# kaiidams/voice100

Hardware: AMD Instinct MI355X
Metric: audio frames/sec (fwd+bwd) asr_en_base, B=32x1024-frame mel (higher is better)
Workload: dtype bf16

## Files before the change

include/voice100_hip.h:

```cpp
#ifndef VOICE100_HIP_H
#define VOICE100_HIP_H

#ifdef __cplusplus
extern "C" {
#endif


int v100_dw_num_groups(int B, int C);
int v100_dwconv(const float* x, const float* x2, const float* w, const float* in_a, const float* in_b,
                const float* in_c, int in_mode, float* y, const float* aux, const float* out_a,
                const float* out_b, int out_mode, float* stats, int G, int B, int C, int Tin, int Tout,
                int K, int stride, int pad, int flip, int upsample, int force_generic, void* stream);

int v100_dwconv_wgrad(const float* g, const float* g2, const float* ga, const float* gb, const float* gc,
                      int g_mode, const float* x, const float* xa, const float* xb, int x_mode,
                      float* partial, float* dw, int G, int B, int C, int Tin, int Tout, int K, int stride,
                      int pad, int force_generic, void* stream);

int v100_dwconv_bwd(const float* g, const float* g2, const float* w, const float* ga, const float* gb,
                    const float* gc, const float* xpre, const float* xa, const float* xb, float* dxin,
                    float* stats, float* wpartial, float* dw, int G, int B, int C, int Tin, int Tout, int K,
                    int stride, int pad, int force_split, void* stream);

int v100_pw_num_parts(int B, int T);
// ... 104 lines not shown
long long v100_launch_count(void);
int v100_copy_probe(const void* src, void* dst, long long nbytes, void* stream);
int v100_timing_enable(int tag_mask);
int v100_timing_read(int tag, double* ms, long long* count, double* bytes);
int v100_rows_copy_probe(const void* src, void* dst, int B, int C, int row_bytes, void* stream);

int v100_pw_gemm_io(const void* A_bf16, const void* X, const void* X2, const float* xa, const float* xb, const float* xc,
                    int x_mode, void* Y, const float* ea, const float* eb, const void* R, int epi_mode, float* stats,
                    int B, int M, int K, int T, int io16, void* stream);
int v100_pw_wgrad_io(const void* G, const void* G2, const float* ga, const float* gb, const float* gc, int g_mode,
                     const void* X, const float* xa, const float* xb, int x_mode, float* partial, float* dW, int S, int B,
                     int M, int K, int T, int io16, void* stream);
int v100_pw_wgrad_group_supported(int B, int M, int K, int T, int S, int g_mode, int x_mode, int io16);
int v100_pw_wgrad_group_tiles(int M, int K, int x_mode);
int v100_pw_wgrad_group(int n, const void* const* ptrs, const int* dims, void* stream);
int v100_dw_mfma_supported(int K, int stride);
int v100_row_pitch16(int T, int B);
int v100_dwconv_fwd_train_io(const void* a1, const float* w, const float* in_a, const float* in_b, void* a2, float* stats,
                             int G, int B, int C, int T, int K, int io16, void* stream);
int v100_dwconv_bwd_io(const void* g, const void* g2, const float* w, const float* ga, const float* gb, const float* gc,
                       const void* xpre, const float* xa, const float* xb, void* dxin, float* stats, float* wpartial,
                       float* dw, int G, int B, int C, int T, int K, int io16, void* stream);
int v100_dwconv_bwd_da1_io(const void* g, const void* g2, const float* w, const float* ga, const float* gb, const float* gc,
                           const void* xpre, const float* xa, const float* xb, void* da1_out, float* stats, float* dw,
                           const float* bn1_gamma, const float* bn1_mean, const float* bn1_rstd, float* pqr, float* dgamma,
                           float* dbeta, int B, int C, int T, int K, void* stream);
int v100_dwconv_fwd_eval_io(const void* h1, const float* w, const float* out_a, const float* out_b, void* h2, int B, int C, int T,
                            int K, int flags, void* stream);
int v100_chan_reduce2_io(const void* u, const void* v, float* partial, int G, int B, int C, int T, int io16, void* stream);
int v100_chan_affine2_shadow(const void* u, const float* v, const float* A, const float* Cc, float* out, void* shadow,
// ... 32 lines not shown
long long v100_ir_eval_cache_bytes(const int* shape);
int v100_ir_eval_prep(const int* shape, const void* const* ptrs, void* stream);
int v100_ir_fwd_eval(const int* shape, const void* const* ptrs, void* stream);
int v100_ir_stack_fwd_eval(int n, const int* shapes, const void* const* ptrs, void* stream);
int v100_ir_prep_batched(const int* shapes, const void* const* w1s, const void* const* w3s, void* const* preps, int n, void* stream);
int v100_ir_fwd_train(const int* shape, const void* const* ptrs, void* stream);
long long v100_ir_bwd_workspace_bytes(const int* shape);
int v100_ir_bwd(const int* shape, const void* const* ptrs, void* stream);

long long v100_ir_stack_plan(const int* desc, long long* plan);
int v100_ir_stack_fwd_train(const int* desc, const void* const* params, const void* x, const void* x16, void* blob, void* stream);
int v100_ir_stack_bwd(const int* desc, const void* const* params, const void* x, const void* x16, const void* blob, const void* dy,
                      void* dx, void* grads, void* ws, void* stream);
int v100_ir_stack_wgrad_plan(const int* desc, int have_x16, int min_problem_tiles, int min_flush_tiles, long long* out);
int v100_ir_stack_wgrad_group_thresholds(int min_problem_tiles, int min_flush_tiles);

int v100_ctc_greedy_decode(const float* logits, const int* lens, long long* out, int* out_len, int B, int T, int V, int blank, void* stream);
int v100_ctc_best_path(const float* logp, const long long* labels, const int* in_len, const int* lab_len, void* back_ws, int* path,
                       float* score, int B, int T, int V, int Lmax, int max_move, void* stream);
long long v100_ctc_align_workspace_bytes(int B, int T, int Lmax);
int v100_ctc_align_block(void);
int v100_ctc_align(const float* logp, const long long* labels, const int* in_len, const int* lab_len, void* moves_ws, int* path,
                   long long* best_labels, int* align, float* score, int B, int T, int V, int Lmax, int max_move, void* stream);
long long v100_edit_distance_workspace_bytes(int B, int Th, int Tr);
int v100_edit_distance(const long long* hyp, const int* hyp_len, const long long* ref, const int* ref_len, void* ws, int* dist,
                       int* hyp_n, int* ref_n, long long* totals, int B, int Th, int Tr, int levels, long long sep, void* stream);
long long v100_ctc_beam_workspace_bytes(int B, int T, int V, int W);
int v100_ctc_beam_search(const float* logits, const int* lens, void* ws, long long* ids, int* ids_len, float* scores, int B, int T, int V,
                         int W, int nbest, int blank, void* stream);
int v100_ctc_beam_search_lm(const float* logits, const int* lens, void* ws, long long* ids, int* ids_len, float* scores,
// ... 86 lines not shown
```

voice100_amd/csrc/block.hip:

```cpp
#include "common.h"
#include "../../include/voice100_hip.h"
#include "depthwise_common.h"
#include "block_shape.h"
#include <algorithm>

static inline size_t al256(size_t v) { return (v + 255) & ~size_t(255); }
static const float kMom = 0.1f, kEps = 1e-5f;
#define CK(call) do { rc = (call); if (rc) return rc; } while (0)

static inline int pitch16(int T, int B) { return v100_pitch16(T, B); }
extern "C" int v100_row_pitch16(int T, int B) { return v100_pitch16(T, B); }
enum { PW_IO_X = 1, PW_IO_X2 = 2, PW_IO_Y = 4, PW_IO_R = 8, PW_IO_F16 = 16, WG_IO_G = 1, WG_IO_G2 = 2, WG_IO_X = 4 };

struct IrBn { const float *gamma, *beta; float *rm, *rv; long long* nbt; };
struct IrBnCoef { float *s, *t, *m, *r; };
struct IrCoef { IrBnCoef bn1, bn2, bn3; };
static IrCoef ir_coef(const float* coef, int mc) {
    float* c = const_cast<float*>(coef);
    return {{c, c + mc, c + 2 * mc, c + 3 * mc}, {c + 4 * mc, c + 5 * mc, c + 6 * mc, c + 7 * mc}, {c + 8 * mc, c + 9 * mc, c + 10 * mc, c + 11 * mc}};
}
struct IrParams { const float* w1; IrBn bn1; const float* wd; IrBn bn2; const float* w3; IrBn bn3; };
static IrParams ir_params(const void* const* t) {
    auto bn = [&](int j) { return IrBn{(const float*)t[j], (const float*)t[j + 1], (float*)t[j + 2], (float*)t[j + 3], (long long*)t[j + 4]}; };
    return {(const float*)t[0], bn(1), (const float*)t[6], bn(7), (const float*)t[12], bn(13)};
// ... 114 lines not shown
    } else {
        w.dz2 = c.take<float>((size_t)B * hid * T2);
        w.dz1 = c.take<float>((size_t)B * hid * T);
    }
    w.slab = c.take<float>(std::max({(size_t)v100_pw_wgrad_splits(B, cout, hid) * cout * hid, (size_t)v100_pw_wgrad_splits(B, hid, cin) * hid * cin,
                                     (size_t)v100_dw_num_groups(B, hid) * hid * K}));
    w.pqr = c.take<float>((size_t)6 * s.mc);
    return c.used + 256;
}

static size_t ir_defer_da3_bytes(const IrShape& s) { return al256((size_t)s.B * s.cout * pitch16(s.T2, s.B) * 2); }
static size_t ir_defer_bytes(const IrShape& s) { return ir_defer_da3_bytes(s) + al256((size_t)s.B * s.hid * pitch16(s.T, s.B) * 2); }
static int ir_wgrad_defer_tiles(const IrShape& s) {
    return v100_pw_wgrad_group_tiles(s.cout, s.hid, 1) + v100_pw_wgrad_group_tiles(s.hid, s.cin, 0);
}
static bool ir_wgrad_defer_ok(const IrShape& s, bool have_x16, int min_tiles) {
    const int B = s.B, cin = s.cin, hid = s.hid, cout = s.cout, T = s.T, K = s.K;
    if (s.act16 < 4 || !s.shadows || s.frozen || !have_x16 || s.S != 1) return false;
    if (!ir_act16_supported(s) || v100_dw_num_groups(B, hid) != 1 || !dw_bwd_da1_supported(B, hid, T, K, 1)) return false;
    const int io = WG_IO_G | WG_IO_X;
    return v100_pw_wgrad_group_supported(B, cout, hid, T, v100_pw_wgrad_splits(B, cout, hid), 0, 1, io) &&
           v100_pw_wgrad_group_supported(B, hid, cin, T, v100_pw_wgrad_splits(B, hid, cin), 0, 0, io) &&
           v100_pw_wgrad_group_tiles(cout, hid, 1) >= min_tiles && v100_pw_wgrad_group_tiles(hid, cin, 0) >= min_tiles;
}

extern "C" long long v100_ir_bwd_workspace_bytes(const int* shape) {
    IrBwdWs w;
    IrShape s = ir_shape(shape, false);
    s.act16 = shape[IR_ACT16];
    return (long long)ir_bwd_carve(s, nullptr, w);
}

static int ir_bwd(const IrShape& s, const IrBwdArgs& a, hipStream_t stream) {
    const int B = s.B, cin = s.cin, hid = s.hid, cout = s.cout, T = s.T, K = s.K, S = s.S, res = s.res, bf = s.bf, pad = s.pad, T2 = s.T2, mc = s.mc;
    const float *x = a.x, *a1 = a.a1, *a2 = a.a2, *a3 = a.a3, *wd = a.wd, *g1 = a.g1, *g2 = a.g2, *g3 = a.g3, *dy = a.dy;
    const IrCoef c = ir_coef(a.coef, mc);
    const float *s1 = c.bn1.s, *t1 = c.bn1.t, *s2 = c.bn2.s, *t2 = c.bn2.t;
    float* dx = a.dx;
// ... 170 lines not shown
}
extern "C" int v100_ir_stack_fwd_eval(int n, const int* shapes, const void* const* ptrs, void* stream) {
    if (!shapes || !ptrs) return V100_ERR_NULL;
    if (n < 0) return V100_ERR_SHAPE;
    int rc;
    for (int i = 0; i < n; ++i, shapes += IR_NSHAPE, ptrs += 8)
        CK(ir_fwd_eval(ir_shape(shapes, false), ir_eval_layout(shapes), ir_eval_args(ptrs), (hipStream_t)stream));
    return V100_OK;
}

enum { ST_N, ST_B, ST_T, ST_BF16, ST_LEVEL, ST_SHADOW, ST_HDR };
namespace {
struct StackBlock { IrShape s; long long a1, a2, a3, y, y16, coef, prep; int Tout; size_t grad_floats; long long defer_off; };
struct StackTotals { size_t blob_bytes, bwd_ws, grad_floats, fwd_ws_off, wsmax, dxmax; };
int wg_min_problem_tiles = 32, wg_min_flush_tiles = 192;
int stack_layout(const int* desc, StackBlock* blk, StackTotals& t, int min_tiles = wg_min_problem_tiles) {
    t = StackTotals{};
    const int n = desc[ST_N], B = desc[ST_B], bf = desc[ST_BF16], level = desc[ST_LEVEL];
    if (n <= 0 || n > 32 || B <= 0 || desc[ST_T] <= 0 || (bf != 0 && bf != 1)) return 0;
    int T = desc[ST_T];
    size_t off = 0, fwd_ws = 0;
    const bool shadows = bf == 1 && level >= 4;
    for (int i = 0; i < n; ++i) {
        const int* d = desc + ST_HDR + 6 * i;
        StackBlock& b = blk[i];
        const int cin = d[0], hid = d[1], cout = d[2], k = d[3], st = d[4], res = d[5];
        if (cin <= 0 || hid <= 0 || cout <= 0 || k <= 0 || st <= 0) return 0;
        const int dims[9] = {B, cin, hid, cout, T, k, st, res, bf};
        IrShape& s = b.s = ir_shape(dims, false);
        s.prepped = true; s.shadows = shadows;
// ... 33 lines not shown
void stack_flush_plan(const StackBlock* blk, int n, bool have_x16, int min_flush, bool* defer, int* flush) {
    int tiles = 0, count = 0;
    for (int i = n - 1; i >= 0; --i) {
        defer[i] = blk[i].defer_off >= 0 && (i > 0 || have_x16);
        flush[i] = 0;
        if (defer[i]) { tiles += ir_wgrad_defer_tiles(blk[i].s); count += 2; }
        if (!count) continue;
        const bool next = i > 0 && blk[i - 1].defer_off >= 0 && (i > 1 || have_x16);
        const bool fits = next && count + 2 <= 16 && tiles + ir_wgrad_defer_tiles(blk[i - 1].s) <= 256;
        if (i == 0 || count + 2 > 16 || (tiles >= min_flush && !fits)) {
            flush[i] = tiles >= min_flush ? tiles : -tiles;
            tiles = count = 0;
        }
    }
}
}

extern "C" int v100_ir_stack_wgrad_group_thresholds(int min_problem_tiles, int min_flush_tiles) {
    if (min_problem_tiles < 1 || min_flush_tiles < 1) return V100_ERR_SHAPE;
    wg_min_problem_tiles = min_problem_tiles;
    wg_min_flush_tiles = min_flush_tiles;
    return V100_OK;
}

extern "C" int v100_ir_stack_wgrad_plan(const int* desc, int have_x16, int min_problem_tiles, int min_flush_tiles, long long* out) {
    if (!desc || !out) return V100_ERR_NULL;
    if (min_problem_tiles < 1 || min_flush_tiles < 1) return V100_ERR_SHAPE;
    StackBlock blk[32];
    StackTotals t;
    if (!stack_layout(desc, blk, t, min_problem_tiles)) return V100_ERR_SHAPE;
    const int n = desc[ST_N];
    bool defer[32]; int flush[32];
    stack_flush_plan(blk, n, have_x16 != 0, min_flush_tiles, defer, flush);
    size_t shared = t.bwd_ws;
    for (int i = 0; i < n; ++i) {
        out[3 * i] = defer[i]; out[3 * i + 1] = blk[i].defer_off; out[3 * i + 2] = flush[i];
        if (blk[i].defer_off >= 0 && (size_t)blk[i].defer_off < shared) shared = (size_t)blk[i].defer_off;
    }
    out[3 * n] = (long long)t.bwd_ws; out[3 * n + 1] = (long long)shared;
    return V100_OK;
}

extern "C" long long v100_ir_stack_plan(const int* desc, long long* plan) {
    if (!desc || !plan) return -1;
    StackBlock blk[32];
    StackTotals t;
    if (!stack_layout(desc, blk, t)) return -1;
    const int n = desc[ST_N];
    for (int i = 0; i < n; ++i) {
        long long* o = plan + 8 * i;
        o[0] = blk[i].a1; o[1] = blk[i].a2; o[2] = blk[i].a3; o[3] = blk[i].y; o[4] = blk[i].y16; o[5] = blk[i].coef; o[6] = blk[i].prep;
        o[7] = blk[i].Tout;
    }
    const long long tot[6] = {(long long)t.blob_bytes, (long long)t.bwd_ws, (long long)t.grad_floats, (long long)t.fwd_ws_off, 0, 0};
// ... 44 lines not shown
    const char* base = (const char*)blob;
    auto at = [&](long long off) { return (const float*)(base + off); };
    char* w0 = (char*)ws;
    char* pp[2] = {w0 + al256(t.wsmax), w0 + al256(t.wsmax) + al256(t.dxmax)};
    size_t goff = t.grad_floats;
    const void* dyi = dy;
    int rc;
    static const bool grad16_on = [] { const char* e = getenv("V100_IR_GRAD16"); return !(e && e[0] == '0'); }();
    auto grad16_ok = [&](int i) {
        const IrShape& s = blk[i].s;
        return grad16_on && desc[ST_LEVEL] >= 5 && s.act16 >= 3 && s.S == 1 && s.T >= 8 && chan_bn3_bwd_fits(s.B, s.T) && ir_act16_supported(s) &&
               dw_bwd_da1_supported(s.B, s.hid, s.T, s.K, v100_dw_num_groups(s.B, s.hid));
    };
    bool defer[32]; int flush[32];
    stack_flush_plan(blk, n, x16 != nullptr, wg_min_flush_tiles, defer, flush);
    const void* gp[5 * 16]; int gd[8 * 16]; int gblk[16]; int ng = 0;
    auto flush_pending = [&](bool grouped) -> int {
        int rc = V100_OK;
        if (grouped) rc = v100_pw_wgrad_group(ng, gp, gd, stream);
        else
            for (int j = 0; j < ng && rc == V100_OK; ++j) {
                IrBwdWs w;
                ir_bwd_carve(blk[gblk[j]].s, w0, w);
                const int* d = gd + 8 * j;
                rc = v100_pw_wgrad_io(gp[5 * j], nullptr, nullptr, nullptr, nullptr, d[5], gp[5 * j + 1], (const float*)gp[5 * j + 2],
                                      (const float*)gp[5 * j + 3], d[6], w.slab, (float*)const_cast<void*>(gp[5 * j + 4]), d[4], d[0], d[1], d[2], d[3],
                                      d[7], stream);
            }
        ng = 0;
        return rc;
    };
    bool dy_is16 = false;
    for (int i = n - 1; i >= 0; --i) {
        const StackBlock& b = blk[i];
        IrShape s = b.s;
        s.defer = defer[i];
        const bool dx_is16 = i > 0 && grad16_ok(i) && grad16_ok(i - 1);
        if (dy_is16 && !grad16_ok(i)) return V100_ERR_SHAPE;
        s.dy16 = dy_is16; s.dx16 = dx_is16;
        goff -= b.grad_floats;
        void* dxi = i > 0 ? (void*)pp[i & 1] : dx;
        const IrParams p = ir_params(params + 18 * i);
        const void* x16i = i > 0 ? (blk[i - 1].y16 >= 0 ? (const void*)(base + blk[i - 1].y16) : nullptr) : x16;
        IrBwdArgs a{i > 0 ? at(blk[i - 1].y) : (const float*)x, at(b.a1), at(b.a2), at(b.a3), p.w1, p.wd, p.w3, p.bn1.gamma, p.bn2.gamma, p.bn3.gamma,
                    at(b.coef), (const float*)dyi, (float*)dxi, {}, w0, (void*)(base + b.prep), x16i, defer[i] ? w0 + b.defer_off : nullptr};
        ir_grads_carve(s, (float*)grads + goff, a.g);
        CK(ir_bwd(s, a, (hipStream_t)stream));
        if (defer[i]) {
            const IrBnCoef bn2 = ir_coef(a.coef, s.mc).bn2;
            char* own = w0 + b.defer_off;
            const void* pr[2][5] = {{own, a.a2, bn2.s, bn2.t, a.g.dW3}, {own + ir_defer_da3_bytes(s), a.x16, nullptr, nullptr, a.g.dW1}};
            const int dm[2][8] = {{s.B, s.cout, s.hid, s.T, v100_pw_wgrad_splits(s.B, s.cout, s.hid), 0, 1, WG_IO_G | WG_IO_X},
                                  {s.B, s.hid, s.cin, s.T, v100_pw_wgrad_splits(s.B, s.hid, s.cin), 0, 0, WG_IO_G | WG_IO_X}};
            for (int j = 0; j < 2; ++j, ++ng) {
                for (int e = 0; e < 5; ++e) gp[5 * ng + e] = pr[j][e];
                for (int e = 0; e < 8; ++e) gd[8 * ng + e] = dm[j][e];
                gblk[ng] = i;
            }
        }
        if (flush[i]) CK(flush_pending(flush[i] > 0));
        dyi = dxi;
        dy_is16 = dx_is16;
    }
    return V100_OK;
}
```

voice100_amd/csrc/pointwise_bf16_group.hip:

```cpp
#include "pointwise_bf16_wgrad_group.h"
#include "timing.h"

extern "C" int v100_pw_wgrad_group_supported(int B, int M, int K, int T, int S, int g_mode, int x_mode, int io16) {
    if (B <= 0 || M <= 0 || K <= 0 || T <= 0 || S <= 0 || (S > B && (S % B != 0 || S / B > 64))) return 0;
    if (g_mode != PW_X_NONE || (x_mode != PW_X_NONE && x_mode != PW_X_AFFINE_RELU6) || io16 != (WG_IO_G | WG_IO_X)) return 0;
    const int GR = x_mode ? 256 : 128, XR = x_mode ? 128 : 256;
    if (M % GR || K % XR) return 0;
    const int P = pw_pitch16(T, B);
    return ((long)(M + 256) * P * 4 < 0x7fffffffL && (long)(K + 256) * P * 4 < 0x7fffffffL) ? 1 : 0;
}

extern "C" int v100_pw_wgrad_group_tiles(int M, int K, int x_mode) {
    const int GR = x_mode ? 256 : 128, XR = x_mode ? 128 : 256;
    return (M > 0 && K > 0 && M % GR == 0 && K % XR == 0) ? (M / GR) * (K / XR) : 0;
}

extern "C" int v100_pw_wgrad_group(int n, const void* const* ptrs, const int* dims, void* stream) {
    if (!ptrs || !dims) return V100_ERR_NULL;
    if (n <= 0 || n > WG_GROUP_MAX) return V100_ERR_SHAPE;
    WgGroupParams g;
    g.n = n;
    int fill[8] = {0, 0, 0, 0, 0, 0, 0, 0};
    bool tail = false;
    for (int i = 0; i < n; ++i) {
        const void* const* P = ptrs + 5 * i;
        const int* d = dims + 8 * i;
        if (!P[0] || !P[1] || !P[4] || (d[6] != PW_X_NONE && (!P[2] || !P[3]))) return V100_ERR_NULL;
        if (!v100_pw_wgrad_group_supported(d[0], d[1], d[2], d[3], d[4], d[5], d[6], d[7])) return V100_ERR_SHAPE;
        WgGroupProblem& q = g.pr[i];
        q.G = P[0]; q.X = P[1]; q.xa = (const float*)P[2]; q.xb = (const float*)P[3]; q.dW = (float*)P[4];
        q.B = d[0]; q.M = d[1]; q.K = d[2]; q.T = d[3]; q.S = d[4]; q.x_mode = d[6];
        q.ntiles = v100_pw_wgrad_group_tiles(q.M, q.K, q.x_mode);
        int x = 0;
        for (int c = 1; c < 8; ++c) if (fill[c] < fill[x]) x = c;
        q.xcd = x; q.slot0 = fill[x];
        fill[x] += q.ntiles;
        tail = tail || q.T % BF_BK != 0;
    }
    int slots = 0;
    for (int c = 0; c < 8; ++c) if (fill[c] > slots) slots = fill[c];
    hipStream_t st = (hipStream_t)stream;
    V100TimedRegion timed(V100_T_PW_WGRAD, st);
    if (tail) V100_GGL((pw_wgrad_group_kernel<true, WG_GROUP_RL>), dim3((unsigned)(8 * slots)), dim3(768), 0, st, g);
    else V100_GGL((pw_wgrad_group_kernel<false, WG_GROUP_RL>), dim3((unsigned)(8 * slots)), dim3(768), 0, st, g);
    return v100_launch_status();
}
```

voice100_amd/csrc/pointwise_bf16_wgrad_group.h:

```cpp
#pragma once
#include "pointwise_bf16_wgrad_ws.h"

struct WgGroupProblem {
    const void* G; const void* X; const float* xa; const float* xb; float* dW;
    int B, M, K, T, S, x_mode;
    int xcd, slot0, ntiles;
};
#define WG_GROUP_MAX 16
#define WG_GROUP_RL 2
struct WgGroupParams { WgGroupProblem pr[WG_GROUP_MAX]; int n; };

template <bool TAIL, int RL>
__global__ __launch_bounds__(768) void pw_wgrad_group_kernel(WgGroupParams g) {
    __shared__ __attribute__((aligned(16))) unsigned char smem[98304 + RL * 32768];
    const int x = blockIdx.x & 7, j = blockIdx.x >> 3;
    int pi = -1;
    for (int i = 0; i < g.n; ++i)
        if (g.pr[i].xcd == x && j >= g.pr[i].slot0 && j < g.pr[i].slot0 + g.pr[i].ntiles) pi = i;
    if (pi < 0) return;
    const WgGroupProblem& q = g.pr[pi];
    const int t = j - q.slot0;
    WgParams p{(const float*)q.G, nullptr, nullptr, nullptr, nullptr, (const float*)q.X, q.xa, q.xb, q.dW, q.B, q.M, q.K, q.T, q.S, 0, q.x_mode,
               0, 0, 0, 0, 0, 0, 0, 0u, WG_IO_G | WG_IO_X};
    f32x4* const runs = reinterpret_cast<f32x4*>(smem + 98304);
    if (q.x_mode == PW_X_AFFINE_RELU6) {
        const int nkt = q.K / 128;
        pw_wgrad_bf16_ws_body<0, 1, TAIL, WG_IO_G | WG_IO_X, 256, 128, 4, true, RL>(p, 0, t / nkt, t % nkt, smem, smem + 65536, runs);
    } else {
        const int nkt = q.K / 256;
        pw_wgrad_bf16_ws_body<0, 0, TAIL, WG_IO_G | WG_IO_X, 128, 256, 4, true, RL>(p, 0, t / nkt, t % nkt, smem, smem + 32768, runs);
    }
}
```

voice100_amd/csrc/pointwise_bf16_wgrad_ws.h:

```cpp
#pragma once
#include "pointwise_bf16_common.h"

template <int GM, int XM, bool TAIL, int IO, int GR, int XR, int NSW, bool GRP = false, int RL = 0>
__device__ __forceinline__ void pw_wgrad_bf16_ws_body(const WgParams& p, const int s, const int mt, const int ktile, unsigned char* const As0,
                                                      unsigned char* const Bs0, f32x4* const runs) {
    static_assert(!(GM != PW_X_NONE && XM != PW_X_NONE), "at most one transformed operand (128 rows); the other one plain (256 rows)");
    static_assert((IO & WG_IO_G) && (IO & WG_IO_X) && (GM != PW_X_AFFINE2 || (IO & WG_IO_G2)), "bf16-stored operands only");
    constexpr bool PG = GM == PW_X_NONE && XM != PW_X_NONE;
    static_assert((PG ? GR : XR) == 256 && (PG ? XR : GR) == 128, "tile shape");
    constexpr int QM = PG ? XM : GM;
    constexpr int NX = XR / 64;
    static_assert(NSW == 4 || NSW == 8, "staging waves: one or two per SIMD");
    constexpr int NSQ = (QM == PW_X_AFFINE2 && NSW == 4) ? 3 : 4;
    constexpr int NQP = 16 / NSW;
    constexpr int QRS = 8 * NSW;
    unsigned char (*As)[GR * 128] = reinterpret_cast<unsigned char (*)[GR * 128]>(As0);
    unsigned char (*Bs)[XR * 128] = reinterpret_cast<unsigned char (*)[XR * 128]>(Bs0);
    const int tid = threadIdx.x, lane = tid & 63;
    const int wave = __builtin_amdgcn_readfirstlane(tid >> 6);
    const int m0 = mt * GR, n0 = ktile * XR;
    const int M = p.M, K = p.K, T = p.T;
    const int P16 = pw_pitch16(T, p.B);
    const int nt = (T + BF_BK - 1) / BF_BK;
    const WgSpan sp = GRP ? WgSpan{0, p.B, 0, nt} : wg_span(p, s, nt);
    const int nsteps = sp.nb * sp.ntl, b_lo = sp.b_lo;
    auto step_bt = [&](int step, int& b, int& t0) {
// ... 1 lines not shown
        (void)q;
        const int bi = q / sp.ntl;
        b = b_lo + bi;
        t0 = (sp.t_first + q - bi * sp.ntl) * BF_BK;
    };
    auto tail_mask = [&](u32x4 v, int tb) {
        const int nv = T - tb;
#pragma unroll
        for (int j = 0; j < 4; ++j) v[j] &= nv > 2 * j + 1 ? 0xffffffffu : (nv > 2 * j ? 0xffffu : 0u);
        return v;
    };
    if (!GRP && nsteps == 0) {
        if (wave < 8) {
            const int wm = wave / NX, wn = wave % NX, col = lane & 31, half = lane >> 5;
#pragma unroll
            for (int i = 0; i < 2; ++i)
#pragma unroll
                for (int j = 0; j < 2; ++j)
#pragma unroll
                    for (int r = 0; r < 16; ++r) {
                        const int m = m0 + wm * 64 + i * 32 + (r & 3) + 8 * (r >> 2) + 4 * half, k = n0 + wn * 64 + j * 32 + col;
                        p.partial[((size_t)s * M + m) * K + k] = 0.f;
                    }
        }
        return;
    }

    if (wave >= 8) {
        const int pt = tid - 512;
        const int qrow = pt >> 3, ch = pt & 7;
        const int row0 = PG ? n0 : m0, rows = PG ? K : M;
        const float* q1 = PG ? p.X : p.G;
        const float* q2 = PG ? p.X : p.G2;
        const float* pa = PG ? p.xa : p.ga;
        const float* pb = PG ? p.xb : p.gb;
        unsigned char (*Qs)[128 * 128] = PG ? reinterpret_cast<unsigned char (*)[128 * 128]>(Bs) : reinterpret_cast<unsigned char (*)[128 * 128]>(As);
// ... 98 lines not shown
                    if (st + 2 < nsteps) {
                        stage(st + 3, S3{});
                        __syncthreads();
                    }
                }
            }
        }
#undef WS_SB
        return;
    }

    const int wm = wave / NX, wn = wave % NX;
    const int prow = tid >> 3, pch = tid & 7;
    const int prow0 = PG ? m0 : n0, prows = PG ? M : K;
    const float* pp = PG ? p.G : p.X;
    unsigned char (*Ps)[256 * 128] = PG ? reinterpret_cast<unsigned char (*)[256 * 128]>(As) : reinterpret_cast<unsigned char (*)[256 * 128]>(Bs);
    const int voP = ((prow0 + prow) * P16 + pch * 8) * 2;
    const int stepP = 64 * P16 * 2;
    const int ldsP = bf_off(prow, pch);
    u32x4 rp[2][4];
    auto load_p = [&](int step, auto stg, int i) {
        constexpr int SG = decltype(stg)::value;
        int b, t0;
        step_bt(step, b, t0);
        const __amdgpu_buffer_rsrc_t r = make_rsrc(reinterpret_cast<const u16*>(pp) + (size_t)b * prows * P16, (unsigned)prows * P16 * 2u);
        rp[SG][i] = __builtin_amdgcn_raw_buffer_load_b128(r, voP, t0 * 2 + i * stepP, 0);
    };
    auto piece_out = [&](int step, u32x4 v) {
        if constexpr (TAIL) {
            int b, t0;
            step_bt(step, b, t0);
            if (t0 + BF_BK > T) v = tail_mask(v, t0 + pch * 8);
        }
        return v;
    };
    f32x16 acc[2][2];
#pragma unroll
    for (int i = 0; i < 2; ++i)
#pragma unroll
        for (int j = 0; j < 2; ++j)
#pragma unroll
            for (int r = 0; r < 16; ++r) acc[i][j][r] = 0.f;
    const int lr = lane & 31, lh = lane >> 5;
    const int sw = (lr >> 1) & 7;
    const int rdA0 = (wm * 64 + lr) * 128, rdB0 = (wn * 64 + lr) * 128;
    auto block = [&](int st, auto stg) {
        constexpr int SG = decltype(stg)::value;
        const unsigned char* Ab = As[st & 1];
        const unsigned char* Bb = Bs[st & 1];
        unsigned char* Pd = Ps[(st + 1) & 1] + ldsP;
#pragma unroll
        for (int ks = 0; ks < BF_BK / 16; ++ks) {
            const int co = ((ks * 2 + lh) ^ sw) << 4;
            const bf16x8 a0 = *reinterpret_cast<const bf16x8*>(Ab + rdA0 + co);
            const bf16x8 a1 = *reinterpret_cast<const bf16x8*>(Ab + rdA0 + 32 * 128 + co);
            const bf16x8 b0 = *reinterpret_cast<const bf16x8*>(Bb + rdB0 + co);
            const bf16x8 b1 = *reinterpret_cast<const bf16x8*>(Bb + rdB0 + 32 * 128 + co);
            acc[0][0] = __builtin_amdgcn_mfma_f32_32x32x16_bf16(a0, b0, acc[0][0], 0, 0, 0);
            acc[0][1] = __builtin_amdgcn_mfma_f32_32x32x16_bf16(a0, b1, acc[0][1], 0, 0, 0);
            acc[1][0] = __builtin_amdgcn_mfma_f32_32x32x16_bf16(a1, b0, acc[1][0], 0, 0, 0);
            acc[1][1] = __builtin_amdgcn_mfma_f32_32x32x16_bf16(a1, b1, acc[1][1], 0, 0, 0);
            __builtin_amdgcn_sched_barrier(0);
            *reinterpret_cast<u32x4*>(Pd + ks * 8192) = piece_out(st + 1, rp[SG][ks]);
            load_p(st + 3, stg, ks);
            __builtin_amdgcn_sched_barrier(0);
        }
    };
    using S0 = std::integral_constant<int, 0>; using S1 = std::integral_constant<int, 1>;
#pragma unroll
    for (int i = 0; i < 4; ++i) load_p(0, S0{}, i);
    __builtin_amdgcn_sched_barrier(0);
#pragma unroll
    for (int i = 0; i < 4; ++i) load_p(1, S1{}, i);
    __builtin_amdgcn_sched_barrier(0);
#pragma unroll
    for (int i = 0; i < 4; ++i) { *reinterpret_cast<u32x4*>(Ps[0] + ldsP + i * 8192) = piece_out(0, rp[0][i]); load_p(2, S0{}, i); }
    __builtin_amdgcn_sched_barrier(0);
    __syncthreads();
    constexpr int NRR = GRP ? 4 - RL : 1;
    f32x16 run[NRR];
    const int per = ((p.B + p.S - 1) / p.S) * sp.ntl, TS = p.S > p.B ? p.S / p.B : 0;
    auto next_fold = [&](int cur) {
        if (TS == 0) return min(cur + per, nsteps);
        const int b = cur / sp.ntl, w = cur - b * sp.ntl;
        int c = 0;
        while ((int)((long)(c + 1) * sp.ntl / TS) <= w) ++c;
        return b * sp.ntl + (int)((long)(c + 1) * sp.ntl / TS);
    };
    int fold_at = GRP ? next_fold(0) : 0;
    if constexpr (GRP) {
#pragma unroll
        for (int f = 0; f < NRR; ++f)
#pragma unroll
            for (int r = 0; r < 16; ++r) run[f][r] = 0.f;
#pragma unroll
        for (int f = 0; f < RL * 4; ++f) runs[f * 512 + tid] = f32x4{0.f, 0.f, 0.f, 0.f};
    }
    auto fold = [&](int done) {
        if constexpr (GRP) {
            if (done != fold_at) return;
            fold_at = next_fold(done);
#pragma unroll
            for (int f = 0; f < 4; ++f) {
                f32x16& a = acc[f >> 1][f & 1];
                if (f < NRR) {
#pragma unroll
                    for (int r = 0; r < 16; ++r) run[f < NRR ? f : 0][r] += a[r];
                } else {
#pragma unroll
                    for (int q = 0; q < 4; ++q) {
                        f32x4& d = runs[((f - NRR) * 4 + q) * 512 + tid];
                        d += f32x4{a[4 * q], a[4 * q + 1], a[4 * q + 2], a[4 * q + 3]};
                    }
                }
#pragma unroll
                for (int r = 0; r < 16; ++r) a[r] = 0.f;
            }
        }
// ... 2 lines not shown
    for (; st + 1 < nsteps; st += 2) {
        block(st, S1{});
        fold(st + 1);
        __syncthreads();
        block(st + 1, S0{});
        fold(st + 2);
        __syncthreads();
    }
    if (st < nsteps) {
        block(st, S1{});
        fold(st + 1);
        __syncthreads();
    }
    const int col = lane & 31, half = lane >> 5;
#pragma unroll
    for (int i = 0; i < 2; ++i)
#pragma unroll
        for (int j = 0; j < 2; ++j)
#pragma unroll
            for (int r = 0; r < 16; ++r) {
                const int m = m0 + wm * 64 + i * 32 + (r & 3) + 8 * (r >> 2) + 4 * half;
                const int k = n0 + wn * 64 + j * 32 + col;
                float v = acc[i][j][r];
                if constexpr (GRP) {
                    const int f = i * 2 + j;
                    v = f < NRR ? run[f < NRR ? f : 0][r] : runs[((f - NRR) * 4 + (r >> 2)) * 512 + tid][r & 3];
                }
                p.partial[((size_t)s * M + m) * K + k] = v;
            }
}

template <int GM, int XM, bool TAIL, int IO, int GR, int XR, int NSW>
__global__ __launch_bounds__(512 + 64 * NSW) void pw_wgrad_bf16_ws_kernel(WgParams p) {
    __shared__ __attribute__((aligned(16))) unsigned char As[2][GR * 128];
    __shared__ __attribute__((aligned(16))) unsigned char Bs[2][XR * 128];
    int s, mt, ktile;
// ... 4 lines not shown
```

Baseline: 10.65 million.

## Add small-tile grouped pointwise wgrad tier with region-lending defer plan

Adds a second tier of deferred weight-gradient grouping for inverted-residual blocks that the existing 256-row-tile grouped kernel rejects. These blocks use a new 128x128-tile grouped kernel, and their deferred gradients borrow freed defer regions from other blocks. The planner lends free regions and schedules separate flushes, so more small per-block wgrad GEMMs are batched into a single grouped launch instead of many small launches. The cost is added planning complexity and smaller tiles with less operand reuse per tile, plus a risk of region aliasing bugs if the lending state is tracked wrongly.

```diff
diff --git a/include/voice100_hip.h b/include/voice100_hip.h
--- a/include/voice100_hip.h
+++ b/include/voice100_hip.h
@@ -142,6 +142,9 @@
 int v100_pw_wgrad_group_supported(int B, int M, int K, int T, int S, int g_mode, int x_mode, int io16);
 int v100_pw_wgrad_group_tiles(int M, int K, int x_mode);
 int v100_pw_wgrad_group(int n, const void* const* ptrs, const int* dims, void* stream);
+int v100_pw_wgrad_group_small_supported(int B, int M, int K, int T, int S, int g_mode, int x_mode, int io16);
+int v100_pw_wgrad_group_small_tiles(int M, int K);
+int v100_pw_wgrad_group_small(int n, const void* const* ptrs, const int* dims, void* stream);
 int v100_dw_mfma_supported(int K, int stride);
 int v100_row_pitch16(int T, int B);
 int v100_dwconv_fwd_train_io(const void* a1, const float* w, const float* in_a, const float* in_b, void* a2, float* stats,
@@ -204,6 +207,9 @@
                       void* dx, void* grads, void* ws, void* stream);
 int v100_ir_stack_wgrad_plan(const int* desc, int have_x16, int min_problem_tiles, int min_flush_tiles, long long* out);
 int v100_ir_stack_wgrad_group_thresholds(int min_problem_tiles, int min_flush_tiles);
+int v100_ir_stack_wgrad_small_plan(const int* desc, int have_x16, int min_problem_tiles, int min_flush_tiles, int min_small_tiles,
+                                   int min_small_flush_tiles, long long* out);
+int v100_ir_stack_wgrad_small_thresholds(int min_problem_tiles, int min_flush_tiles);
 
 int v100_ctc_greedy_decode(const float* logits, const int* lens, long long* out, int* out_len, int B, int T, int V, int blank, void* stream);
 int v100_ctc_best_path(const float* logp, const long long* labels, const int* in_len, const int* lab_len, void* back_ws, int* path,
diff --git a/voice100_amd/csrc/block.hip b/voice100_amd/csrc/block.hip
--- a/voice100_amd/csrc/block.hip
+++ b/voice100_amd/csrc/block.hip
@@ -152,14 +152,28 @@
 static int ir_wgrad_defer_tiles(const IrShape& s) {
     return v100_pw_wgrad_group_tiles(s.cout, s.hid, 1) + v100_pw_wgrad_group_tiles(s.hid, s.cin, 0);
 }
+static bool ir_wgrad_defer_path(const IrShape& s, bool have_x16) {
+    if (s.act16 < 4 || !s.shadows || s.frozen || !have_x16 || s.S != 1) return false;
+    return ir_act16_supported(s) && v100_dw_num_groups(s.B, s.hid) == 1 && dw_bwd_da1_supported(s.B, s.hid, s.T, s.K, 1);
+}
 static bool ir_wgrad_defer_ok(const IrShape& s, bool have_x16, int min_tiles) {
-    const int B = s.B, cin = s.cin, hid = s.hid, cout = s.cout, T = s.T, K = s.K;
-    if (s.act16 < 4 || !s.shadows || s.frozen || !have_x16 || s.S != 1) return false;
-    if (!ir_act16_supported(s) || v100_dw_num_groups(B, hid) != 1 || !dw_bwd_da1_supported(B, hid, T, K, 1)) return false;
+    const int B = s.B, cin = s.cin, hid = s.hid, cout = s.cout, T = s.T;
+    if (!ir_wgrad_defer_path(s, have_x16)) return false;
     const int io = WG_IO_G | WG_IO_X;
     return v100_pw_wgrad_group_supported(B, cout, hid, T, v100_pw_wgrad_splits(B, cout, hid), 0, 1, io) &&
            v100_pw_wgrad_group_supported(B, hid, cin, T, v100_pw_wgrad_splits(B, hid, cin), 0, 0, io) &&
            v100_pw_wgrad_group_tiles(cout, hid, 1) >= min_tiles && v100_pw_wgrad_group_tiles(hid, cin, 0) >= min_tiles;
+}
+static int ir_wgrad_defer_small_tiles(const IrShape& s) {
+    return v100_pw_wgrad_group_small_tiles(s.cout, s.hid) + v100_pw_wgrad_group_small_tiles(s.hid, s.cin);
+}
+static bool ir_wgrad_defer_small_ok(const IrShape& s, bool have_x16, int min_tiles) {
+    const int B = s.B, cin = s.cin, hid = s.hid, cout = s.cout, T = s.T;
+    if (!ir_wgrad_defer_path(s, have_x16)) return false;
+    const int io = WG_IO_G | WG_IO_X;
+    return v100_pw_wgrad_group_small_supported(B, cout, hid, T, v100_pw_wgrad_splits(B, cout, hid), 0, 1, io) &&
+           v100_pw_wgrad_group_small_supported(B, hid, cin, T, v100_pw_wgrad_splits(B, hid, cin), 0, 0, io) &&
+           v100_pw_wgrad_group_small_tiles(cout, hid) >= min_tiles && v100_pw_wgrad_group_small_tiles(hid, cin) >= min_tiles;
 }
 
 extern "C" long long v100_ir_bwd_workspace_bytes(const int* shape) {
@@ -360,6 +374,7 @@
 struct StackBlock { IrShape s; long long a1, a2, a3, y, y16, coef, prep; int Tout; size_t grad_floats; long long defer_off; };
 struct StackTotals { size_t blob_bytes, bwd_ws, grad_floats, fwd_ws_off, wsmax, dxmax; };
 int wg_min_problem_tiles = 32, wg_min_flush_tiles = 192;
+int wg_min_small_tiles = 16, wg_min_small_flush_tiles = 128;
 int stack_layout(const int* desc, StackBlock* blk, StackTotals& t, int min_tiles = wg_min_problem_tiles) {
     t = StackTotals{};
     const int n = desc[ST_N], B = desc[ST_B], bf = desc[ST_BF16], level = desc[ST_LEVEL];
@@ -423,12 +438,52 @@
         }
     }
 }
+
+void stack_small_plan(const StackBlock* blk, int n, bool have_x16, const bool* defer, const int* flush, int min_tiles, int min_flush,
+                      bool* defer2, int* region, int* flush2) {
+    enum { HELD, FREE, LENT };
+    int state[32];
+    for (int i = 0; i < n; ++i) state[i] = HELD;
+    auto pick = [&](int i) {
+        if (defer[i] || !ir_wgrad_defer_small_ok(blk[i].s, i > 0 ? blk[i - 1].y16 >= 0 : have_x16, min_tiles)) return -1;
+        for (int j = n - 1; j >= 0; --j)
+            if (state[j] == FREE && ir_defer_bytes(blk[j].s) >= ir_defer_bytes(blk[i].s)) return j;
+        return -1;
+    };
+    int tiles = 0, count = 0, pending1 = 0;
+    int wait1[32];
+    for (int i = n - 1; i >= 0; --i) {
+        defer2[i] = false; region[i] = -1; flush2[i] = 0;
+        const int r = pick(i);
+        if (r >= 0) {
+            defer2[i] = true; region[i] = r; state[r] = LENT;
+            tiles += ir_wgrad_defer_small_tiles(blk[i].s); count += 2;
+        }
+        if (defer[i]) wait1[pending1++] = i;
+        if (flush[i]) { while (pending1) state[wait1[--pending1]] = FREE; }
+        if (!count) continue;
+        const int nr = i > 0 ? pick(i - 1) : -1;
+        const bool fits = nr >= 0 && count + 2 <= 16 && tiles + ir_wgrad_defer_small_tiles(blk[i - 1].s) <= 256;
+        if (i == 0 || count + 2 > 16 || (tiles >= min_flush && !fits)) {
+            flush2[i] = tiles >= min_flush ? tiles : -tiles;
+            tiles = count = 0;
+            for (int j = 0; j < n; ++j) if (state[j] == LENT) state[j] = FREE;
+        }
+    }
+}
 }
 
 extern "C" int v100_ir_stack_wgrad_group_thresholds(int min_problem_tiles, int min_flush_tiles) {
     if (min_problem_tiles < 1 || min_flush_tiles < 1) return V100_ERR_SHAPE;
     wg_min_problem_tiles = min_problem_tiles;
     wg_min_flush_tiles = min_flush_tiles;
+    return V100_OK;
+}
+
+extern "C" int v100_ir_stack_wgrad_small_thresholds(int min_problem_tiles, int min_flush_tiles) {
+    if (min_problem_tiles < 1 || min_flush_tiles < 1) return V100_ERR_SHAPE;
+    wg_min_small_tiles = min_problem_tiles;
+    wg_min_small_flush_tiles = min_flush_tiles;
     return V100_OK;
 }
 
@@ -447,6 +502,25 @@
         if (blk[i].defer_off >= 0 && (size_t)blk[i].defer_off < shared) shared = (size_t)blk[i].defer_off;
     }
     out[3 * n] = (long long)t.bwd_ws; out[3 * n + 1] = (long long)shared;
+    return V100_OK;
+}
+
+extern "C" int v100_ir_stack_wgrad_small_plan(const int* desc, int have_x16, int min_problem_tiles, int min_flush_tiles, int min_small_tiles,
+                                              int min_small_flush_tiles, long long* out) {
+    if (!desc || !out) return V100_ERR_NULL;
+    if (min_problem_tiles < 1 || min_flush_tiles < 1 || min_small_tiles < 1 || min_small_flush_tiles < 1) return V100_ERR_SHAPE;
+    StackBlock blk[32];
+    StackTotals t;
+    if (!stack_layout(desc, blk, t, min_problem_tiles)) return V100_ERR_SHAPE;
+    const int n = desc[ST_N];
+    bool defer[32], defer2[32]; int flush[32], region[32], flush2[32];
+    stack_flush_plan(blk, n, have_x16 != 0, min_flush_tiles, defer, flush);
+    stack_small_plan(blk, n, have_x16 != 0, defer, flush, min_small_tiles, min_small_flush_tiles, defer2, region, flush2);
+    for (int i = 0; i < n; ++i) {
+        out[4 * i] = defer2[i]; out[4 * i + 1] = region[i];
+        out[4 * i + 2] = region[i] >= 0 ? blk[region[i]].defer_off : -1; out[4 * i + 3] = flush2[i];
+    }
+    out[4 * n] = (long long)t.bwd_ws;
     return V100_OK;
 }
 
@@ -521,27 +595,33 @@
     };
     bool defer[32]; int flush[32];
     stack_flush_plan(blk, n, x16 != nullptr, wg_min_flush_tiles, defer, flush);
-    const void* gp[5 * 16]; int gd[8 * 16]; int gblk[16]; int ng = 0;
-    auto flush_pending = [&](bool grouped) -> int {
+    bool defer2[32]; int region[32], flush2[32];
+    stack_small_plan(blk, n, x16 != nullptr, defer, flush, wg_min_small_tiles, wg_min_small_flush_tiles, defer2, region, flush2);
+    struct Pending { const void* gp[5 * 16]; int gd[8 * 16]; int gblk[16]; int ng; };
+    Pending pend[2];
+    pend[0].ng = pend[1].ng = 0;
+    auto flush_pending = [&](int tier, bool grouped) -> int {
+        Pending& q = pend[tier];
         int rc = V100_OK;
-        if (grouped) rc = v100_pw_wgrad_group(ng, gp, gd, stream);
+        if (grouped) rc = (tier ? v100_pw_wgrad_group_small : v100_pw_wgrad_group)(q.ng, q.gp, q.gd, stream);
         else
-            for (int j = 0; j < ng && rc == V100_OK; ++j) {
+            for (int j = 0; j < q.ng && rc == V100_OK; ++j) {
                 IrBwdWs w;
-                ir_bwd_carve(blk[gblk[j]].s, w0, w);
-                const int* d = gd + 8 * j;
-                rc = v100_pw_wgrad_io(gp[5 * j], nullptr, nullptr, nullptr, nullptr, d[5], gp[5 * j + 1], (const float*)gp[5 * j + 2],
-                                      (const float*)gp[5 * j + 3], d[6], w.slab, (float*)const_cast<void*>(gp[5 * j + 4]), d[4], d[0], d[1], d[2], d[3],
-                                      d[7], stream);
+                ir_bwd_carve(blk[q.gblk[j]].s, w0, w);
+                const int* d = q.gd + 8 * j;
+                rc = v100_pw_wgrad_io(q.gp[5 * j], nullptr, nullptr, nullptr, nullptr, d[5], q.gp[5 * j + 1], (const float*)q.gp[5 * j + 2],
+                                      (const float*)q.gp[5 * j + 3], d[6], w.slab, (float*)const_cast<void*>(q.gp[5 * j + 4]), d[4], d[0], d[1], d[2],
+                                      d[3], d[7], stream);
             }
-        ng = 0;
+        q.ng = 0;
         return rc;
     };
     bool dy_is16 = false;
     for (int i = n - 1; i >= 0; --i) {
         const StackBlock& b = blk[i];
         IrShape s = b.s;
-        s.defer = defer[i];
+        s.defer = defer[i] || defer2[i];
+        char* const own = !s.defer ? nullptr : w0 + (defer[i] ? b.defer_off : blk[region[i]].defer_off);
         const bool dx_is16 = i > 0 && grad16_ok(i) && grad16_ok(i - 1);
         if (dy_is16 && !grad16_ok(i)) return V100_ERR_SHAPE;
         s.dy16 = dy_is16; s.dx16 = dx_is16;
@@ -550,22 +630,23 @@
         const IrParams p = ir_params(params + 18 * i);
         const void* x16i = i > 0 ? (blk[i - 1].y16 >= 0 ? (const void*)(base + blk[i - 1].y16) : nullptr) : x16;
         IrBwdArgs a{i > 0 ? at(blk[i - 1].y) : (const float*)x, at(b.a1), at(b.a2), at(b.a3), p.w1, p.wd, p.w3, p.bn1.gamma, p.bn2.gamma, p.bn3.gamma,
-                    at(b.coef), (const float*)dyi, (float*)dxi, {}, w0, (void*)(base + b.prep), x16i, defer[i] ? w0 + b.defer_off : nullptr};
+                    at(b.coef), (const float*)dyi, (float*)dxi, {}, w0, (void*)(base + b.prep), x16i, own};
         ir_grads_carve(s, (float*)grads + goff, a.g);
         CK(ir_bwd(s, a, (hipStream_t)stream));
-        if (defer[i]) {
+        if (s.defer) {
             const IrBnCoef bn2 = ir_coef(a.coef, s.mc).bn2;
-            char* own = w0 + b.defer_off;
+            Pending& q = pend[defer[i] ? 0 : 1];
             const void* pr[2][5] = {{own, a.a2, bn2.s, bn2.t, a.g.dW3}, {own + ir_defer_da3_bytes(s), a.x16, nullptr, nullptr, a.g.dW1}};
             const int dm[2][8] = {{s.B, s.cout, s.hid, s.T, v100_pw_wgrad_splits(s.B, s.cout, s.hid), 0, 1, WG_IO_G | WG_IO_X},
                                   {s.B, s.hid, s.cin, s.T, v100_pw_wgrad_splits(s.B, s.hid, s.cin), 0, 0, WG_IO_G | WG_IO_X}};
-            for (int j = 0; j < 2; ++j, ++ng) {
-                for (int e = 0; e < 5; ++e) gp[5 * ng + e] = pr[j][e];
-                for (int e = 0; e < 8; ++e) gd[8 * ng + e] = dm[j][e];
-                gblk[ng] = i;
+            for (int j = 0; j < 2; ++j, ++q.ng) {
+                for (int e = 0; e < 5; ++e) q.gp[5 * q.ng + e] = pr[j][e];
+                for (int e = 0; e < 8; ++e) q.gd[8 * q.ng + e] = dm[j][e];
+                q.gblk[q.ng] = i;
             }
         }
-        if (flush[i]) CK(flush_pending(flush[i] > 0));
+        if (flush[i]) CK(flush_pending(0, flush[i] > 0));
+        if (flush2[i]) CK(flush_pending(1, flush2[i] > 0));
         dyi = dxi;
         dy_is16 = dx_is16;
     }
diff --git a/voice100_amd/csrc/pointwise_bf16_group.hip b/voice100_amd/csrc/pointwise_bf16_group.hip
--- a/voice100_amd/csrc/pointwise_bf16_group.hip
+++ b/voice100_amd/csrc/pointwise_bf16_group.hip
@@ -15,7 +15,18 @@
     return (M > 0 && K > 0 && M % GR == 0 && K % XR == 0) ? (M / GR) * (K / XR) : 0;
 }
 
-extern "C" int v100_pw_wgrad_group(int n, const void* const* ptrs, const int* dims, void* stream) {
+extern "C" int v100_pw_wgrad_group_small_supported(int B, int M, int K, int T, int S, int g_mode, int x_mode, int io16) {
+    if (B <= 0 || M <= 0 || K <= 0 || T <= 0 || S <= 0 || (S > B && (S % B != 0 || S / B > 64))) return 0;
+    if (g_mode != PW_X_NONE || (x_mode != PW_X_NONE && x_mode != PW_X_AFFINE_RELU6) || io16 != (WG_IO_G | WG_IO_X)) return 0;
+    if (M % 128 || K % 128) return 0;
+    const int P = pw_pitch16(T, B);
+    return ((long)(M + 256) * P * 4 < 0x7fffffffL && (long)(K + 256) * P * 4 < 0x7fffffffL) ? 1 : 0;
+}
+extern "C" int v100_pw_wgrad_group_small_tiles(int M, int K) {
+    return (M > 0 && K > 0 && M % 128 == 0 && K % 128 == 0) ? (M / 128) * (K / 128) : 0;
+}
+
+static int wgrad_group_launch(int n, const void* const* ptrs, const int* dims, void* stream, bool small) {
     if (!ptrs || !dims) return V100_ERR_NULL;
     if (n <= 0 || n > WG_GROUP_MAX) return V100_ERR_SHAPE;
     WgGroupParams g;
@@ -26,11 +37,12 @@
         const void* const* P = ptrs + 5 * i;
         const int* d = dims + 8 * i;
         if (!P[0] || !P[1] || !P[4] || (d[6] != PW_X_NONE && (!P[2] || !P[3]))) return V100_ERR_NULL;
-        if (!v100_pw_wgrad_group_supported(d[0], d[1], d[2], d[3], d[4], d[5], d[6], d[7])) return V100_ERR_SHAPE;
+        if (!(small ? v100_pw_wgrad_group_small_supported : v100_pw_wgrad_group_supported)(d[0], d[1], d[2], d[3], d[4], d[5], d[6], d[7]))
+            return V100_ERR_SHAPE;
         WgGroupProblem& q = g.pr[i];
         q.G = P[0]; q.X = P[1]; q.xa = (const float*)P[2]; q.xb = (const float*)P[3]; q.dW = (float*)P[4];
         q.B = d[0]; q.M = d[1]; q.K = d[2]; q.T = d[3]; q.S = d[4]; q.x_mode = d[6];
-        q.ntiles = v100_pw_wgrad_group_tiles(q.M, q.K, q.x_mode);
+        q.ntiles = small ? v100_pw_wgrad_group_small_tiles(q.M, q.K) : v100_pw_wgrad_group_tiles(q.M, q.K, q.x_mode);
         int x = 0;
         for (int c = 1; c < 8; ++c) if (fill[c] < fill[x]) x = c;
         q.xcd = x; q.slot0 = fill[x];
@@ -41,7 +53,19 @@
     for (int c = 0; c < 8; ++c) if (fill[c] > slots) slots = fill[c];
     hipStream_t st = (hipStream_t)stream;
     V100TimedRegion timed(V100_T_PW_WGRAD, st);
-    if (tail) V100_GGL((pw_wgrad_group_kernel<true, WG_GROUP_RL>), dim3((unsigned)(8 * slots)), dim3(768), 0, st, g);
-    else V100_GGL((pw_wgrad_group_kernel<false, WG_GROUP_RL>), dim3((unsigned)(8 * slots)), dim3(768), 0, st, g);
+    const dim3 grid((unsigned)(8 * slots));
+    if (small) {
+        if (tail) V100_GGL((pw_wgrad_group_small_kernel<true>), grid, dim3(768), 0, st, g);
+        else V100_GGL((pw_wgrad_group_small_kernel<false>), grid, dim3(768), 0, st, g);
+    } else {
+        if (tail) V100_GGL((pw_wgrad_group_kernel<true, WG_GROUP_RL>), grid, dim3(768), 0, st, g);
+        else V100_GGL((pw_wgrad_group_kernel<false, WG_GROUP_RL>), grid, dim3(768), 0, st, g);
+    }
     return v100_launch_status();
 }
+extern "C" int v100_pw_wgrad_group(int n, const void* const* ptrs, const int* dims, void* stream) {
+    return wgrad_group_launch(n, ptrs, dims, stream, false);
+}
+extern "C" int v100_pw_wgrad_group_small(int n, const void* const* ptrs, const int* dims, void* stream) {
+    return wgrad_group_launch(n, ptrs, dims, stream, true);
+}
diff --git a/voice100_amd/csrc/pointwise_bf16_wgrad_group.h b/voice100_amd/csrc/pointwise_bf16_wgrad_group.h
--- a/voice100_amd/csrc/pointwise_bf16_wgrad_group.h
+++ b/voice100_amd/csrc/pointwise_bf16_wgrad_group.h
@@ -31,3 +31,21 @@
         pw_wgrad_bf16_ws_body<0, 0, TAIL, WG_IO_G | WG_IO_X, 128, 256, 4, true, RL>(p, 0, t / nkt, t % nkt, smem, smem + 32768, runs);
     }
 }
+
+template <bool TAIL>
+__global__ __launch_bounds__(768) void pw_wgrad_group_small_kernel(WgGroupParams g) {
+    __shared__ __attribute__((aligned(16))) unsigned char smem[65536];
+    const int x = blockIdx.x & 7, j = blockIdx.x >> 3;
+    int pi = -1;
+    for (int i = 0; i < g.n; ++i)
+        if (g.pr[i].xcd == x && j >= g.pr[i].slot0 && j < g.pr[i].slot0 + g.pr[i].ntiles) pi = i;
+    if (pi < 0) return;
+    const WgGroupProblem& q = g.pr[pi];
+    const int t = j - q.slot0, nkt = q.K / 128;
+    WgParams p{(const float*)q.G, nullptr, nullptr, nullptr, nullptr, (const float*)q.X, q.xa, q.xb, q.dW, q.B, q.M, q.K, q.T, q.S, 0, q.x_mode,
+               0, 0, 0, 0, 0, 0, 0, 0u, WG_IO_G | WG_IO_X};
+    if (q.x_mode == PW_X_AFFINE_RELU6)
+        pw_wgrad_bf16_ws_body<0, 1, TAIL, WG_IO_G | WG_IO_X, 128, 128, 4, true, 0>(p, 0, t / nkt, t % nkt, smem, smem + 32768, nullptr);
+    else
+        pw_wgrad_bf16_ws_body<0, 0, TAIL, WG_IO_G | WG_IO_X, 128, 128, 4, true, 0>(p, 0, t / nkt, t % nkt, smem, smem + 32768, nullptr);
+}
diff --git a/voice100_amd/csrc/pointwise_bf16_wgrad_ws.h b/voice100_amd/csrc/pointwise_bf16_wgrad_ws.h
--- a/voice100_amd/csrc/pointwise_bf16_wgrad_ws.h
+++ b/voice100_amd/csrc/pointwise_bf16_wgrad_ws.h
@@ -7,9 +7,14 @@
     static_assert(!(GM != PW_X_NONE && XM != PW_X_NONE), "at most one transformed operand (128 rows); the other one plain (256 rows)");
     static_assert((IO & WG_IO_G) && (IO & WG_IO_X) && (GM != PW_X_AFFINE2 || (IO & WG_IO_G2)), "bf16-stored operands only");
     constexpr bool PG = GM == PW_X_NONE && XM != PW_X_NONE;
-    static_assert((PG ? GR : XR) == 256 && (PG ? XR : GR) == 128, "tile shape");
+    constexpr int PR = PG ? GR : XR;
+    static_assert((PR == 256 || (PR == 128 && GRP)) && (PG ? XR : GR) == 128, "tile shape");
     constexpr int QM = PG ? XM : GM;
     constexpr int NX = XR / 64;
+    constexpr int NPP = PR / 64;
+    constexpr int AI = PR == 256 ? 2 : 1;
+    constexpr int NF = AI * 2;
+    static_assert(RL <= NF - 1, "at least one running-sum fragment in registers");
     static_assert(NSW == 4 || NSW == 8, "staging waves: one or two per SIMD");
     constexpr int NSQ = (QM == PW_X_AFFINE2 && NSW == 4) ? 3 : 4;
     constexpr int NQP = 16 / NSW;
@@ -41,12 +46,12 @@
         if (wave < 8) {
             const int wm = wave / NX, wn = wave % NX, col = lane & 31, half = lane >> 5;
 #pragma unroll
-            for (int i = 0; i < 2; ++i)
+            for (int i = 0; i < AI; ++i)
 #pragma unroll
                 for (int j = 0; j < 2; ++j)
 #pragma unroll
                     for (int r = 0; r < 16; ++r) {
-                        const int m = m0 + wm * 64 + i * 32 + (r & 3) + 8 * (r >> 2) + 4 * half, k = n0 + wn * 64 + j * 32 + col;
+                        const int m = m0 + wm * (32 * AI) + i * 32 + (r & 3) + 8 * (r >> 2) + 4 * half, k = n0 + wn * 64 + j * 32 + col;
                         p.partial[((size_t)s * M + m) * K + k] = 0.f;
                     }
         }
@@ -175,11 +180,11 @@
     const int prow = tid >> 3, pch = tid & 7;
     const int prow0 = PG ? m0 : n0, prows = PG ? M : K;
     const float* pp = PG ? p.G : p.X;
-    unsigned char (*Ps)[256 * 128] = PG ? reinterpret_cast<unsigned char (*)[256 * 128]>(As) : reinterpret_cast<unsigned char (*)[256 * 128]>(Bs);
+    unsigned char (*Ps)[PR * 128] = PG ? reinterpret_cast<unsigned char (*)[PR * 128]>(As) : reinterpret_cast<unsigned char (*)[PR * 128]>(Bs);
     const int voP = ((prow0 + prow) * P16 + pch * 8) * 2;
     const int stepP = 64 * P16 * 2;
     const int ldsP = bf_off(prow, pch);
-    u32x4 rp[2][4];
+    u32x4 rp[2][NPP];
     auto load_p = [&](int step, auto stg, int i) {
         constexpr int SG = decltype(stg)::value;
         int b, t0;
@@ -195,50 +200,82 @@
         }
         return v;
     };
-    f32x16 acc[2][2];
-#pragma unroll
-    for (int i = 0; i < 2; ++i)
+    f32x16 acc[AI][2];
+#pragma unroll
+    for (int i = 0; i < AI; ++i)
 #pragma unroll
         for (int j = 0; j < 2; ++j)
 #pragma unroll
             for (int r = 0; r < 16; ++r) acc[i][j][r] = 0.f;
     const int lr = lane & 31, lh = lane >> 5;
     const int sw = (lr >> 1) & 7;
-    const int rdA0 = (wm * 64 + lr) * 128, rdB0 = (wn * 64 + lr) * 128;
+    const int rdA0 = (wm * (32 * AI) + lr) * 128, rdB0 = (wn * 64 + lr) * 128;
     auto block = [&](int st, auto stg) {
         constexpr int SG = decltype(stg)::value;
         const unsigned char* Ab = As[st & 1];
         const unsigned char* Bb = Bs[st & 1];
         unsigned char* Pd = Ps[(st + 1) & 1] + ldsP;
+        if constexpr (AI == 1) {
+            bf16x8 fa[BF_BK / 16], fb[BF_BK / 16][2];
+#pragma unroll
+            for (int ks = 0; ks < BF_BK / 16; ++ks) {
+                const int co = ((ks * 2 + lh) ^ sw) << 4;
+                fa[ks] = *reinterpret_cast<const bf16x8*>(Ab + rdA0 + co);
+                fb[ks][0] = *reinterpret_cast<const bf16x8*>(Bb + rdB0 + co);
+                fb[ks][1] = *reinterpret_cast<const bf16x8*>(Bb + rdB0 + 32 * 128 + co);
+            }
+            __builtin_amdgcn_sched_barrier(0);
+#pragma unroll
+            for (int ks = 0; ks < BF_BK / 16; ++ks) {
+                acc[0][0] = __builtin_amdgcn_mfma_f32_32x32x16_bf16(fa[ks], fb[ks][0], acc[0][0], 0, 0, 0);
+                acc[0][1] = __builtin_amdgcn_mfma_f32_32x32x16_bf16(fa[ks], fb[ks][1], acc[0][1], 0, 0, 0);
+                __builtin_amdgcn_sched_barrier(0);
+                if (ks % 2 == 0) {
+                    *reinterpret_cast<u32x4*>(Pd + (ks / 2) * 8192) = piece_out(st + 1, rp[SG][ks / 2]);
+                    load_p(st + 3, stg, ks / 2);
+                }
+                __builtin_amdgcn_sched_barrier(0);
+            }
+            return;
+        }
 #pragma unroll
         for (int ks = 0; ks < BF_BK / 16; ++ks) {
             const int co = ((ks * 2 + lh) ^ sw) << 4;
             const bf16x8 a0 = *reinterpret_cast<const bf16x8*>(Ab + rdA0 + co);
-            const bf16x8 a1 = *reinterpret_cast<const bf16x8*>(Ab + rdA0 + 32 * 128 + co);
+            bf16x8 a1;
+            if constexpr (AI == 2) a1 = *reinterpret_cast<const bf16x8*>(Ab + rdA0 + 32 * 128 + co);
             const bf16x8 b0 = *reinterpret_cast<const bf16x8*>(Bb + rdB0 + co);
             const bf16x8 b1 = *reinterpret_cast<const bf16x8*>(Bb + rdB0 + 32 * 128 + co);
-            acc[0][0] = __builtin_amdgcn_mfma_f32_32x32x16_bf16(a0, b0, acc[0][0], 0, 0, 0);
-            acc[0][1] = __builtin_amdgcn_mfma_f32_32x32x16_bf16(a0, b1, acc[0][1], 0, 0, 0);
-            acc[1][0] = __builtin_amdgcn_mfma_f32_32x32x16_bf16(a1, b0, acc[1][0], 0, 0, 0);
-            acc[1][1] = __builtin_amdgcn_mfma_f32_32x32x16_bf16(a1, b1, acc[1][1], 0, 0, 0);
+            if constexpr (AI == 2) {
+                acc[0][0] = __builtin_amdgcn_mfma_f32_32x32x16_bf16(a0, b0, acc[0][0], 0, 0, 0);
+                acc[0][1] = __builtin_amdgcn_mfma_f32_32x32x16_bf16(a0, b1, acc[0][1], 0, 0, 0);
+                acc[AI - 1][0] = __builtin_amdgcn_mfma_f32_32x32x16_bf16(a1, b0, acc[AI - 1][0], 0, 0, 0);
+                acc[AI - 1][1] = __builtin_amdgcn_mfma_f32_32x32x16_bf16(a1, b1, acc[AI - 1][1], 0, 0, 0);
+            } else {
+                acc[0][0] = __builtin_amdgcn_mfma_f32_32x32x16_bf16(a0, b0, acc[0][0], 0, 0, 0);
+                acc[0][1] = __builtin_amdgcn_mfma_f32_32x32x16_bf16(a0, b1, acc[0][1], 0, 0, 0);
+            }
             __builtin_amdgcn_sched_barrier(0);
-            *reinterpret_cast<u32x4*>(Pd + ks * 8192) = piece_out(st + 1, rp[SG][ks]);
-            load_p(st + 3, stg, ks);
+            if (ks % (4 / NPP) == 0) {
+                const int pc = ks / (4 / NPP);
+                *reinterpret_cast<u32x4*>(Pd + pc * 8192) = piece_out(st + 1, rp[SG][pc]);
+                load_p(st + 3, stg, pc);
+            }
             __builtin_amdgcn_sched_barrier(0);
         }
     };
     using S0 = std::integral_constant<int, 0>; using S1 = std::integral_constant<int, 1>;
 #pragma unroll
-    for (int i = 0; i < 4; ++i) load_p(0, S0{}, i);
+    for (int i = 0; i < NPP; ++i) load_p(0, S0{}, i);
     __builtin_amdgcn_sched_barrier(0);
 #pragma unroll
-    for (int i = 0; i < 4; ++i) load_p(1, S1{}, i);
+    for (int i = 0; i < NPP; ++i) load_p(1, S1{}, i);
     __builtin_amdgcn_sched_barrier(0);
 #pragma unroll
-    for (int i = 0; i < 4; ++i) { *reinterpret_cast<u32x4*>(Ps[0] + ldsP + i * 8192) = piece_out(0, rp[0][i]); load_p(2, S0{}, i); }
+    for (int i = 0; i < NPP; ++i) { *reinterpret_cast<u32x4*>(Ps[0] + ldsP + i * 8192) = piece_out(0, rp[0][i]); load_p(2, S0{}, i); }
     __builtin_amdgcn_sched_barrier(0);
     __syncthreads();
-    constexpr int NRR = GRP ? 4 - RL : 1;
+    constexpr int NRR = GRP ? NF - RL : 1;
     f32x16 run[NRR];
     const int per = ((p.B + p.S - 1) / p.S) * sp.ntl, TS = p.S > p.B ? p.S / p.B : 0;
     auto next_fold = [&](int cur) {
@@ -262,7 +299,7 @@
             if (done != fold_at) return;
             fold_at = next_fold(done);
 #pragma unroll
-            for (int f = 0; f < 4; ++f) {
+            for (int f = 0; f < NF; ++f) {
                 f32x16& a = acc[f >> 1][f & 1];
                 if (f < NRR) {
 #pragma unroll
@@ -295,12 +332,12 @@
     }
     const int col = lane & 31, half = lane >> 5;
 #pragma unroll
-    for (int i = 0; i < 2; ++i)
+    for (int i = 0; i < AI; ++i)
 #pragma unroll
         for (int j = 0; j < 2; ++j)
 #pragma unroll
             for (int r = 0; r < 16; ++r) {
-                const int m = m0 + wm * 64 + i * 32 + (r & 3) + 8 * (r >> 2) + 4 * half;
+                const int m = m0 + wm * (32 * AI) + i * 32 + (r & 3) + 8 * (r >> 2) + 4 * half;
                 const int k = n0 + wn * 64 + j * 32 + col;
                 float v = acc[i][j][r];
                 if constexpr (GRP) {
```

After: 10.83 million, median of 5. 1.7% higher.
